# robustrobotics/flame

Hardware: AMD Instinct MI355X
Metric: NLTGV2 primal-dual iters/sec on 640x480 Delaunay graph; depth RMS vs CPU (higher is better)
Workload: dtype f32

## Files before the change

flame_amd/csrc/flame_nltgv2_test_options.h:

```cpp
#ifndef FLAME_NLTGV2_TEST_OPTIONS_H_
#define FLAME_NLTGV2_TEST_OPTIONS_H_

enum {
  FLAME_NLTGV2_OPT_BLOCK_WAVES = 103,
  FLAME_NLTGV2_OPT_UNROLL = 104,
  FLAME_NLTGV2_OPT_DUAL_PUBLISH = 106,
  FLAME_NLTGV2_OPT_PRESLEEP = 108,
  FLAME_NLTGV2_OPT_XCDS = 109,
  FLAME_NLTGV2_OPT_FAULT_INJECT = 110,
  FLAME_NLTGV2_OPT_POLL_GAP = 113
};

#endif
```

flame_amd/csrc/nltgv2_context.hip:

```cpp
#include "nltgv2_context.hpp"

namespace flame_hip {
namespace host {

int fail(flame_nltgv2_ctx* ctx, int status) {
  if (ctx) ctx->last_error = status;
  return status;
}

void request_open_stop(flame_nltgv2_ctx* ctx) {
  if (!ctx->open_inflight || ctx->open_stop_sent || !ctx->stop_dev.p || !ctx->ctl_stream) return;
  *ctx->h_stop = ctx->open_tag0;
  if (hipMemcpyAsync(ctx->stop_dev.p, ctx->h_stop, sizeof(unsigned), hipMemcpyHostToDevice, ctx->ctl_stream) != hipSuccess) (void)hipGetLastError();
  ctx->open_stop_sent = true;
}

hipError_t wait_solver_stream(flame_nltgv2_ctx* ctx) {
  request_open_stop(ctx);
  return hipStreamSynchronize(ctx->stream);
}

int ensure(flame_nltgv2_ctx* ctx, DevBuf& b, size_t bytes) {
  if (bytes == 0) bytes = 16;
  if (b.cap >= bytes) return 0;
// ... 442 lines not shown
  ok = ok && hipEventCreateWithFlags(&ctx->ev_snap, hipEventDisableTiming) == hipSuccess;
  ok = ok && hipEventCreateWithFlags(&ctx->ev_raster_done, hipEventDisableTiming) == hipSuccess;
  ok = ok && hipEventCreateWithFlags(&ctx->ev_topo_ready, hipEventDisableTiming) == hipSuccess;
  ok = ok && hipEventCreate(&ctx->ev_mesh0) == hipSuccess && hipEventCreate(&ctx->ev_mesh1) == hipSuccess;
  ok = ok && hipEventCreate(&ctx->ev_dbg0) == hipSuccess && hipEventCreate(&ctx->ev_dbg1) == hipSuccess;
  ok = ok && hipEventCreateWithFlags(&ctx->ev_expanded, hipEventDisableTiming) == hipSuccess;
  ok = ok && hipEventCreateWithFlags(&ctx->ev_run[0], hipEventDisableTiming) == hipSuccess;
  ok = ok && hipEventCreateWithFlags(&ctx->ev_run[1], hipEventDisableTiming) == hipSuccess;
  ok = ok && hipHostMalloc((void**)&ctx->h_err, kErrBytes, hipHostMallocDefault) == hipSuccess;
  ok = ok && hipHostMalloc((void**)&ctx->h_cost, 2 * sizeof(float), hipHostMallocDefault) == hipSuccess;
  ok = ok && hipHostMalloc((void**)&ctx->h_stop, 64, hipHostMallocDefault) == hipSuccess;
  if (ctx->h_stop) *ctx->h_stop = 0u;
  ok = ok && hipStreamCreateWithPriority(&ctx->ctl_stream, hipStreamNonBlocking, -1) == hipSuccess;
  if (!ok) {
    flame_nltgv2_destroy(ctx);
    return FLAME_NLTGV2_ERR_HIP;
  }
  ctx->stream = ctx->own_stream;
  *ctx->h_err = 0;
  {
    static std::once_flag warm;
    if (!std::getenv("FLAME_NLTGV2_NO_WARM"))
    std::call_once(warm, [ctx] {
      warm_module_kernels(), warm_module_persistent(ctx->own_stream, cooperative_allowed()), warm_module_persistent_tv(), warm_module_persistent_pv2();
      warm_module_layout(), warm_module_topo();
    });
    if (!std::getenv("FLAME_NLTGV2_LAZY_CALIBRATION") && ctx->prop.multiProcessorCount >= 64 && place_calibrate_at_create(device) && place_calibrate(ctx) != 0) {
      ctx->last_error = 0, ctx->last_hip = 0;
      (void)hipGetLastError();
    }
    if (ctx->place_state < 0) ctx->place_state = 0;
  }
  ctx->all = {&ctx->pos, &ctx->x, &ctx->w1, &ctx->w2, &ctx->xb, &ctx->w1b, &ctx->w2b, &ctx->xp, &ctx->w1p,
              &ctx->w2p, &ctx->data, &ctx->weight, &ctx->src, &ctx->dst, &ctx->alpha, &ctx->beta, &ctx->q1,
              &ctx->q2, &ctx->q3, &ctx->row_ptr, &ctx->half, &ctx->slice_row, &ctx->perm, &ctx->pdeg,
              &ctx->rec_nbr, &ctx->rec_edge, &ctx->edge_src_slot, &ctx->hrec, &ctx->hq, &ctx->vstate, &ctx->hq_alt, &ctx->vstate_alt, &ctx->cost_terms, &ctx->run_tail,
              &ctx->vaux, &ctx->bar0, &ctx->bar1, &ctx->vprev, &ctx->xbuf, &ctx->abort_flag, &ctx->tv_slot, &ctx->tv_vid, &ctx->tv_meta, &ctx->tv_wave, &ctx->wg2_slot, &ctx->wg2_vid, &ctx->wg2_meta, &ctx->wg2_nbr, &ctx->wg2_fetch, &ctx->wg2_info, &ctx->wg2_vfirst, &ctx->wg2_rmax, &ctx->err,
              &ctx->cost_out, &ctx->img_ref, &ctx->img_cmp, &ctx->photo_err, &ctx->r_tris, &ctx->r_valid, &ctx->r_tvalid, &ctx->r_keys,
              &ctx->r_img, &ctx->r_cov, &ctx->r_vtx, &ctx->r_val, &ctx->wg_slot, &ctx->wg_vid, &ctx->wg_meta, &ctx->wg_nbr,
              &ctx->wg_fetch, &ctx->wg_info, &ctx->wg_v0, &ctx->probe, &ctx->snap_hq, &ctx->snap_vstate, &ctx->snap_bar, &ctx->iperm,
              &ctx->order_m, &ctx->rid_of, &ctx->stage[0].d, &ctx->stage[1].d, &ctx->sync_init, &ctx->sync_vmap, &ctx->sync_emap, &ctx->sync_need,
              &ctx->wg_vfirst, &ctx->place_pool, &ctx->place_rank, &ctx->place_fill, &ctx->place_rec_off, &ctx->place_patch, &ctx->place_meas, &ctx->progress};
  for (DevBuf* b : {&ctx->feat_stamp_d, &ctx->feat_key_d, &ctx->feat_val_d, &ctx->topo_scratch, &ctx->topo_dims, &ctx->layout_pos}) ctx->all.push_back(b);
  for (auto& b : ctx->nx) ctx->all.push_back(&b);
  for (auto& b : ctx->ex) ctx->all.push_back(&b);
  ctx->all.push_back(&ctx->pos_undo);
  for (DevBuf* b : {&ctx->m_P, &ctx->m_idepth, &ctx->m_normals, &ctx->m_tvalid, &ctx->m_nvalid, &ctx->m_tnormal, &ctx->m_offset, &ctx->m_cursor,
// ... 89 lines not shown
      if (value != 2) ctx->persist_refused_topo = ctx->persist_backoff_topo = ~0ull;
      return 0;
    case FLAME_NLTGV2_OPT_PROBE:
      ctx->opt_probe = value ? 1 : 0;
      return 0;
    case FLAME_NLTGV2_OPT_DUAL_PUBLISH:
      if (value < 0 || value > 2) return fail(ctx, FLAME_NLTGV2_ERR_INVALID_ARG);
      ctx->opt_dual = value;
      return 0;
    case FLAME_NLTGV2_OPT_FAULT_INJECT:
      if (value < 0 || value > (1 << 24)) return fail(ctx, FLAME_NLTGV2_ERR_INVALID_ARG);
      ctx->opt_fault = value;
      if (value == 0) ctx->persist_refused_topo = ctx->persist_backoff_topo = ~0ull;
      return 0;
    case FLAME_NLTGV2_OPT_XCDS:
      if (value < 0 || value > 8) return fail(ctx, FLAME_NLTGV2_ERR_INVALID_ARG);
      ctx->opt_xcds = value;
      ctx->coop_checked_key = ~0ull;
      return 0;
    case FLAME_NLTGV2_OPT_PRESLEEP:
      if (value < 0 || value > 256) return fail(ctx, FLAME_NLTGV2_ERR_INVALID_ARG);
      ctx->opt_presleep = value;
      return 0;
    case FLAME_NLTGV2_OPT_MESH_STATE:
      if (value < 0 || value > 1) return fail(ctx, FLAME_NLTGV2_ERR_INVALID_ARG);
      ctx->opt_mesh_state = value;
      return 0;
    case FLAME_NLTGV2_OPT_COST_SUM:
      if (value < 0 || value > 1) return fail(ctx, FLAME_NLTGV2_ERR_INVALID_ARG);
      ctx->opt_cost_sum = value;
      return 0;
    case FLAME_NLTGV2_OPT_SYNC_PATH:
      if (value < 0 || value > 2) return fail(ctx, FLAME_NLTGV2_ERR_INVALID_ARG);
      ctx->opt_sync_path = value;
      return 0;
    case FLAME_NLTGV2_OPT_UNROLL:
      if (value != 0 && value != 4 && value != 8 && value != 16) return fail(ctx, FLAME_NLTGV2_ERR_INVALID_ARG);
      ctx->opt_unroll = value;
      return 0;
    default:
      return fail(ctx, FLAME_NLTGV2_ERR_INVALID_ARG);
  }
}


int flame_nltgv2_get_info(flame_nltgv2_ctx* ctx, flame_nltgv2_info* info) {
// ... 182 lines not shown
```

flame_amd/csrc/nltgv2_context.hpp:

```cpp
#ifndef FLAME_AMD_NLTGV2_CONTEXT_HPP_
#define FLAME_AMD_NLTGV2_CONTEXT_HPP_

#include <hip/hip_runtime.h>

#include <cstdio>
#include <cstdlib>
#include <cstring>
#include <algorithm>
#include <chrono>
#include <cmath>
#include <new>
#include <memory>
#include <mutex>
#include <functional>
#include <vector>

#include "flame_nltgv2.h"
#include "flame_nltgv2_test_options.h"
#include "nltgv2_kernels.h"
#include "nltgv2_pack.hpp"
#include "roctx_ranges.hpp"

namespace flame_hip {
namespace host {
// ... 106 lines not shown
  FlatMap feat_maps[3];
  int feat_cur = 0;
  bool feat_map_valid = false;
  std::vector<int32_t> feat_tab;
  std::vector<uint32_t> feat_stamp;
  uint32_t feat_stamp_now = 0;
  bool feat_tab_valid = false;
  int parity = 0;
  uint64_t topo = 0, stamp = 0;

  int opt_solver = 0, opt_use_graph = 1, opt_block_waves = 0, opt_unroll = 0, opt_persistent = 1, opt_dual = 1;
  int xbuf_form = 0;
  int opt_xcds = 0;
  bool photo_fused = false;
  PhotoGeometry photo_geo{};
  float photo_scale = 1.0f;
  int photo_border = 3;
  bool photo_fresh = false;
  float* export_ptr = nullptr;
  float export_scale = 1.0f;
  int opt_fault = 0;
  int opt_presleep = 0;
  int opt_poll_gap = 0;
  mutable int pv_occ = 0;
  mutable uint64_t pv_occ_topo = ~0ull;
  int opt_probe = 0;
  size_t probe_words = 0;
  uint32_t tag_next = 1;
  int last_run_path = 0, last_run_groups = 0;
  uint64_t persist_refused_topo = ~0ull;
  uint64_t persist_backoff_topo = ~0ull;
  int persist_backoff_left = 0, persist_timeout_streak = 0;
  int replaying = 0;
  uint64_t crowded_until_topo = 0;
  int last_run_waves_per_cu = 0;
  bool static_stale = false;
  uint64_t coop_checked_key = 0;
  int buf_gen = 0;
  int replay_attempt = 0;
  int replays_per_step = 0;
  int timeouts_recovered = 0;
  int torn_records_detected = 0;
  int opt_verify = 0;
  int opt_place = 1;
  int place_state = 0;
  uint64_t place_topo = ~0ull;
// ... 270 lines not shown
```

flame_amd/csrc/nltgv2_kernels.h:

```cpp
#pragma once

#include <hip/hip_runtime.h>
#include <hip/hip_ext.h>
#include <stdint.h>

namespace flame_hip {

struct SolverParams {
  float data_factor, step_x, step_q, theta, x_min, x_max;
};

struct PhotoGeometry {
  float KRKinv[9];
  float Kt[3];
};

struct PhotoFuse {
  const float2* pos = nullptr;
  const uint8_t* ref = nullptr;
  const uint8_t* cmp = nullptr;
  float* err = nullptr;
  PhotoGeometry geo{};
  float graph_scale = 1.0f;
  int rows = 0, cols = 0, step = 0, border = 0;
// ... 124 lines not shown
  const uint32_t* half = nullptr;
  const float2* pos = nullptr;
  float *alpha = nullptr, *beta = nullptr;
  uint8_t* need_nbr = nullptr;
};
int launch_sync_state(const SyncArgs& a, hipStream_t s);
int pv_patches_per_cu(const FusedArgs& a, bool verify);
struct Pv2Args {
  const int32_t* slot = nullptr;
  const int32_t* vid = nullptr;
  const uint32_t* meta = nullptr;
  const int32_t* nbr = nullptr;
  const int32_t* fetch = nullptr;
  const int32_t* info = nullptr;
  int count = 0, lcap = 0;
};
int launch_build_patches2(const CanonArgs& c, const FusedArgs& a, int n_patches, int32_t* wg_info, const int32_t* order_m, const int32_t* rid_tab,
                          const uint8_t* vfirst, const int32_t* iperm, int32_t* wg_slot, int32_t* wg_vid, uint32_t* wg_meta, int32_t* wg_nbr,
                          int32_t* wg_fetch, int* rmax, hipStream_t s);
int pv2_patches_per_cu(int lcap, bool verify);
int launch_persistent_pv2(const FusedArgs& a, const Pv2Args& w, const SolverParams& p, int wg_begin, int n_wgs, int parity_in, unsigned tag0,
                          int n_iters, unsigned max_spins, int poll_gap, int dual, const RunTail* tail, bool cooperative, hipStream_t stream);
int pv_real_waves_per_simd(bool verify_or_probe);
const void* persistent_tv_kernel(int waves_per_block, unsigned* lds_bytes);
int launch_build_sell(const CanonArgs& c, const FusedArgs& a, const int32_t* iperm, hipStream_t s);
int launch_build_patches(const CanonArgs& c, const FusedArgs& a, const int32_t* wg_v0, const int32_t* order_m,
                         const int32_t* rid_tab, const uint8_t* vfirst, const int32_t* iperm, hipStream_t s);
struct TopoDims {
  int32_t n_edges;
  int32_t n_keep;
  int32_t rows;
  int32_t max_degree;
  int32_t wg_count, wg_lcap;
  int32_t wg2_count, wg2_lcap;
  int32_t flags;
  int32_t pad_[7];
};
constexpr int32_t kTopoBadDegree = 1;
constexpr int32_t kTopoBadEdges = 2;
constexpr int kTopoInf = 0x7f7f7f7f;
struct TopoBuild {
  int V = 0, E = 0;
  int Vo = 0, Eo = 0;
  int n_slices = 0;
  const int32_t* fid = nullptr;
  const float2* pos = nullptr;
// ... 21 lines not shown
  void* sort_tmp = nullptr;
  size_t sort_tmp_bytes = 0;
  int* counters = nullptr;
  int32_t* old_of_new = nullptr;
  int32_t* old_of_new_edge = nullptr;
  int32_t *src = nullptr, *dst = nullptr;
  int32_t* row_ptr = nullptr;
  uint32_t* half = nullptr;
  int32_t *order_m = nullptr, *rid_of = nullptr, *perm = nullptr, *iperm = nullptr, *pdeg = nullptr, *slice_row = nullptr;
  int32_t *wg_info = nullptr, *wg_v0 = nullptr, *wg2_info = nullptr, *wg2_v0 = nullptr;
  uint8_t *wg_vfirst = nullptr, *wg2_vfirst = nullptr;
  TopoDims* dims = nullptr;
};
size_t topo_sort_temp_bytes(int V, int n_scan);
int launch_topo_feat_build(const int32_t* feat, int V, uint32_t* stamp, int32_t* key, int32_t* val, int tab_bits, uint32_t gen, hipStream_t s);
int launch_topo_sync_front(const TopoBuild& t, hipStream_t s);
int launch_topo_upload_front(const TopoBuild& t, hipStream_t s);
int launch_topo_back(const TopoBuild& t, hipStream_t s);

void warm_module_kernels();
void warm_module_persistent(hipStream_t stream, bool cooperative);
void warm_module_persistent_tv();
void warm_module_persistent_pv2();
void warm_module_layout();
void warm_module_topo();

int launch_save_prev(const CanonArgs& c, hipStream_t s);
int launch_dual(const CanonArgs& c, const SolverParams& p, hipStream_t s);
int launch_primal(const CanonArgs& c, const SolverParams& p, hipStream_t s);
int launch_extragradient(const CanonArgs& c, const SolverParams& p, hipStream_t s);
int launch_pack_static(const CanonArgs& c, const FusedArgs& a, hipStream_t s);
int launch_pack_state(const CanonArgs& c, const FusedArgs& a, int parity, bool with_static, hipStream_t s);
int launch_unpack_state(const CanonArgs& c, const FusedArgs& a, int parity, bool have_prev, hipStream_t s);
int launch_export(const CanonArgs& c, const FusedArgs& a, bool packed_current, float scale, float* dst,
                  hipStream_t s);
int launch_project_graph(const CanonArgs& c, float graph_scale, const ProjectGeometry& geo, uint8_t* keep, float2* pos_before, hipStream_t s);
int launch_rescale(const CanonArgs& c, float graph_scale, float* new_scale_dev, hipStream_t s);
int launch_interpolate_mesh(int T, const int32_t* tris, const float2* vtx, const float* values, float value_scale,
                            const uint8_t* vtx_valid, const uint8_t* tri_valid, unsigned long long* keys, float* img,
                            int* coverage, int rows, int cols, hipStream_t s);
int launch_photo_residual(const CanonArgs& c, float graph_scale, const PhotoGeometry& geo, const uint8_t* ref,
                          const uint8_t* cmp, int rows, int cols, int step, int border, float* err, hipStream_t s);
int launch_photo_residual_packed(const FusedArgs& a, const PhotoFuse& photo, hipStream_t s);
int launch_cost_terms(const CanonArgs& c, float* terms, hipStream_t s);
int launch_cost_sums(const CanonArgs& c, const float* terms, float* out2, hipStream_t s);

// ... 2 lines not shown
```

flame_amd/csrc/nltgv2_run.hip:

```cpp
#include "nltgv2_context.hpp"

namespace flame_hip {
namespace host {

void pick_config(const flame_nltgv2_ctx* ctx, int* unroll, int* wpb) {
  const bool small = ctx->L.n_slices <= 8 * ctx->prop.multiProcessorCount;
  *unroll = ctx->opt_unroll ? ctx->opt_unroll : (small ? 8 : 4);
  *wpb = ctx->opt_block_waves ? ctx->opt_block_waves : (small ? 1 : 4);
}

struct WaveGroup {
  int begin, count;
};

int ensure_form_rows(flame_nltgv2_ctx* ctx, int form);
int plan_groups(flame_nltgv2_ctx* ctx, int form, int total, int cap, const std::vector<int32_t>& cw, std::vector<WaveGroup>* groups);

bool cooperative_allowed() {
  static const bool ok = [] {
    if (std::getenv("FLAME_NLTGV2_NO_COOPERATIVE")) return false;
    if (std::getenv("FLAME_NLTGV2_COOPERATIVE")) return true;
    if (std::getenv("ROCP_TOOL_LIBRARIES")) return false;
    if (void* h = dlopen("librocprofiler-sdk.so.1", RTLD_NOLOAD | RTLD_LAZY)) {
      dlclose(h);
      return false;
    }
    return true;
  }();
  return ok;
}

int plan_persistent(flame_nltgv2_ctx* ctx, int n, std::vector<WaveGroup>* groups, bool consume = false) {
  groups->clear();
  if (!ctx->opt_persistent || n < 4 || n > (1 << 24) || !ctx->prop.cooperativeLaunch) return 0;
  if (ctx->persist_refused_topo == ctx->topo || ctx->replaying == 2) return 0;
  const bool retry = ctx->replaying == 1;
  if (!retry && ctx->persist_backoff_topo == ctx->topo && (ctx->persist_backoff_left > 0 || ctx->opt_fault > 0)) {
    if (consume && ctx->persist_backoff_left > 0) --ctx->persist_backoff_left;
    return 0;
  }
  PackedLayout& L = ctx->L;
  const int cus = ctx->prop.multiProcessorCount;
  const uint64_t occ_key = ctx->topo * 4 + (ctx->opt_verify != 0 ? 1 : 0) + (ctx->opt_probe != 0 ? 2 : 0);
  if (L.wg_ok && ctx->pv_occ_topo != occ_key) {
    ctx->pv_occ = std::min(kPvDensePerCu, pv_patches_per_cu(ctx->f, ctx->opt_verify != 0 || ctx->opt_probe != 0));
    if (std::getenv("FLAME_NLTGV2_TRACE"))
      std::fprintf(stderr, "[flame_nltgv2] pv: %d patches, row-packed %d, slab slots %d, local records %d -> %d resident per CU\n", L.wg_count,
                   (int)L.wg_rowpack, ctx->f.wg_slab_slots, ctx->f.wg_lcap, ctx->pv_occ);
    ctx->pv_occ_topo = occ_key;
  }
  const bool crowded = (ctx->topo < ctx->crowded_until_topo && ctx->opt_persistent == 1) || retry;
  const int wg_cap = (crowded ? std::min(ctx->pv_occ, kCrowdedWavesPerCu) : ctx->pv_occ) * cus;
  const bool pv_fits = L.wg_ok && L.wg_rowpack && L.wg_count > 0 && L.wg_count <= wg_cap;
  int form = 0;
  auto pv2_usable = [&]() -> bool {
    if (!ctx->wg2_built) return false;
    if (ctx->wg2_checked_topo != ctx->topo) {
// ... 374 lines not shown
    HIPCHK(ctx, hipEventRecord(ctx->ev_snap, ctx->stream));
    ctx->snap_topo = ctx->topo;
  }
  int rc = ensure_fused(ctx);
  if (rc) return rc;
  if (ctx->pending.active) {
    if (ctx->pending.ops.size() >= kMaxChain) {
      rc = finish(ctx);
    } else {
      rc = snapshot_chain_start(ctx);
    }
    if (rc) return rc;
  }
  int unroll, wpb;
  pick_config(ctx, &unroll, &wpb);
  std::vector<WaveGroup> groups;
  const int form = plan_persistent(ctx, n, &groups, true);
  const bool open_run = ctx->want_open != 0 && open_run_applies(ctx, form, groups) && !ctx->pending.active && ctx->opt_probe == 0 &&
                        ctx->opt_verify == 0 && ctx->replaying == 0 && (n & 1) == 0 && ctx->h_stop != nullptr && ctx->ctl_stream != nullptr;
  if (ctx->want_open != 0 && !open_run) {
    ctx->want_open = 0;
    return 0;
  }
  if (form != 0) {
    if ((uint64_t)ctx->tag_next + (uint64_t)n >= 0x07ff0000ull || (ctx->xbuf_form != 0 && ctx->xbuf_form != form)) {
      const size_t bytes = kXbufBytesPerVertex * records_capacity(ctx->L);
      HIPCHK(ctx, hipMemsetAsync(ctx->xbuf.p, 0, bytes, ctx->stream));
      if (ctx->place_base) {
        HIPCHK(ctx, hipMemsetAsync(ctx->place_base, 0, (size_t)2 * kPlacePages * 4096, ctx->stream));
        HIPCHK(ctx, hipMemsetAsync((int*)ctx->place_fill.p + 2 * kPlacePages, 0, 64, ctx->stream));
      }
      HIPCHK(ctx, hipMemsetAsync((int*)ctx->err.p + 12, 0, 2 * sizeof(int), ctx->stream));
      ctx->tag_next = 1;
    }
    ctx->xbuf_form = form;
    const uint32_t tag0 = ctx->tag_next + 2;
    const uint64_t key = ctx->topo * 1024 + (uint64_t)form * 64 + (ctx->opt_verify != 0 ? 16 : 0) + (ctx->opt_probe != 0 ? 8 : 0) +
                         (ctx->opt_dual == 2 ? 4 : ctx->opt_dual == 1 ? 2 : 0) + (ctx->opt_xcds > 0 ? 1 : 0);
    const RunTail* tail_dev = nullptr;
    {
      RunTail want;
      std::memset(static_cast<void*>(&want), 0, sizeof want);
      want.export_out = ctx->export_ptr, want.export_scale = ctx->export_scale;
      if (open_run) {
        const bool fresh = ctx->stop_dev.p == nullptr;
        rc = ensure(ctx, ctx->stop_dev, 64);
        if (rc) return rc;
        if (fresh) HIPCHK(ctx, hipMemsetAsync(ctx->stop_dev.p, 0, 64, ctx->stream));
        ctx->open_tag0 = tag0;
      }
      want.stop_req = open_run ? (const unsigned*)ctx->stop_dev.p : nullptr;
      const PhotoFuse pf = photo_target(ctx);
      std::memcpy(static_cast<void*>(&want.photo), &pf, sizeof pf);
      if (form == 3 && std::getenv("FLAME_NLTGV2_TRACE")) {
        rc = ensure(ctx, ctx->progress, 2 * sizeof(unsigned) * (size_t)ctx->L.wg_count);
        if (rc) return rc;
        HIPCHK(ctx, hipMemsetAsync(ctx->progress.p, 0, 2 * sizeof(unsigned) * (size_t)ctx->L.wg_count, ctx->stream));
        want.progress = (unsigned*)ctx->progress.p;
      }
      constexpr size_t kTailStride = (sizeof(RunTail) + 255) / 256 * 256;
      rc = ensure(ctx, ctx->run_tail, kTailStride * flame_nltgv2_ctx::kTailSlots);
// ... 46 lines not shown
          }
        }
        ctx->f.probe = nullptr;
        if (ctx->opt_probe) {
          const size_t words = (size_t)ctx->L.wg_count * (size_t)n * 8;
          rc = ensure(ctx, ctx->probe, words * sizeof(unsigned));
          if (rc) return rc;
          ctx->f.probe = (unsigned*)ctx->probe.p;
          ctx->probe_words = words;
          HIPCHK(ctx, hipMemsetAsync(ctx->probe.p, 0, words * sizeof(unsigned), ctx->stream));
        }
      }
      if (form == 4) {
        const bool dense = gr.count > kPv2PaceAbovePerCu * ctx->prop.multiProcessorCount;
        const int gap = ctx->opt_poll_gap > 0 ? ctx->opt_poll_gap - 1 : dense ? (3 | ((kPv2DenseGap - 1) << 4)) : kPvPollGap;
        const int poll_gap = gap | ((ctx->opt_presleep > 0 ? ctx->opt_presleep - 1 : dense ? kPv2DensePreSleep : kPvPreSleep) << 8);
        ctx->f.open_run = open_run ? 1 : 0;
        e = launch_persistent_pv2(ctx->f, ctx->pv2_args, to_sp(p), gr.begin, gr.count, ctx->parity, tag0, n, spins_arg, poll_gap, dual,
                                  tail_dev, cooperative_allowed() && ctx->coop_checked_key != key, ctx->stream);
        ctx->f.open_run = 0;
        if (e != 0) break;
        continue;
      }
      ctx->f.open_run = open_run ? 1 : 0;
      e = launch_persistent_run(ctx->f, to_sp(p), form, gr.begin, gr.count, ctx->parity, tag0, n, pw, spins_arg, presleep, dual,
                                xcds, tail_dev, cooperative_allowed() && ctx->coop_checked_key != key, ctx->stream);
      ctx->f.open_run = 0;
      if (e != 0) break;
    }
    ctx->run_event_bound = e == 0 && ctx->f.stop_event != nullptr;
    ctx->f.stop_event = nullptr;
    ctx->tag_next = tag0 + (uint32_t)n;
    if (e == 0) {
      if (!ctx->pending.active) {
        ctx->pending.active = true, ctx->pending.snapshotted = false;
        ctx->pending.ops.clear();
        ctx->pending.parity_before = ctx->parity, ctx->pending.have_prev_before = ctx->have_prev;
      }
      {
        flame_nltgv2_ctx::PendingOp op;
        op.kind = 0, op.params = *p, op.n = n;
        op.open = open_run, op.tag0 = tag0;
        op.dst = ctx->export_ptr, op.scale = ctx->export_scale;
        ctx->pending.ops.push_back(op);
      }
      ctx->photo_fresh = photo_target(ctx).err != nullptr;
// ... 405 lines not shown
```

flame_amd/regularizer.py:

```python
from __future__ import annotations

import ctypes as C
import os

import numpy as np

_HERE = os.path.dirname(os.path.abspath(__file__))
_LIB = None

_FP = C.POINTER(C.c_float)
_IP = C.POINTER(C.c_int32)

OPT_SOLVER, OPT_USE_HIPGRAPH, OPT_PERSISTENT, OPT_PROBE, OPT_VERIFY_RECORDS, OPT_PLACEMENT, OPT_SYNC_PATH, OPT_COST_SUM, OPT_MESH_STATE = 1, 2, 5, 12, 14, 16, 17, 18, 19
OPT_BLOCK_WAVES, OPT_UNROLL, OPT_DUAL_PUBLISH, OPT_PRESLEEP, OPT_XCDS, OPT_FAULT_INJECT, OPT_POLL_GAP = 103, 104, 106, 108, 109, 110, 113
RUN_PATHS = {0: "none", 1: "persistent (the lane-per-half-edge form, retired in round 3)", 2: "per-step hipGraph", 3: "per-step eager", 4: "canonical 4-sweep",
             5: "persistent-tv", 6: "persistent-pv", 7: "persistent-pv2"}
ERR_NAN = -5

VERTEX_STATE = ("x", "w1", "w2", "x_bar", "w1_bar", "w2_bar", "x_prev", "w1_prev", "w2_prev")
EDGE_STATE = ("q1", "q2", "q3")


def _rows_contiguous_u8(a) -> bool:
    return a.dtype == np.uint8 and a.ndim == 2 and a.strides[1] == 1 and a.strides[0] >= max(a.shape[1], 1)


class NLTGV2Error(RuntimeError):
    def __init__(self, status: int, what: str):
        super().__init__(f"{what}: status {status} ({status_string(status)})")
        self.status = status


class Params(C.Structure):

    _fields_ = [(n, C.c_float) for n in ("data_factor", "step_x", "step_q", "theta", "x_min", "x_max")]

    def __init__(self, data_factor=0.1, step_x=0.001, step_q=125.0, theta=0.25, x_min=0.0, x_max=10.0):
# ... 631 lines not shown
```

Baseline: 1.074 million.

## Add lean single-wave persistent PV kernel with inline-asm polling and DPP reductions

Adds a new persistent primal-dual kernel that runs one 64-lane wave per workgroup. The per-iteration loop is hand-written inline assembly: neighbour records are fetched with global_load_lds, readiness is polled on tags held in LDS, and the degree sums use DPP adds. The host selects it by default for form 3 when there is a single wave group, dual publish is on, max degree is at most 16 and occupancy allows. It is meant to cut the per-iteration synchronisation and instruction overhead of the generic persistent kernel. In exchange it adds a large hand-scheduled asm path that is hard to maintain, and correctness depends on its clobber lists and tag handling.

After: 1.142 million, median of 6. +6.3%, better.

```diff
diff --git a/flame_amd/csrc/flame_nltgv2_test_options.h b/flame_amd/csrc/flame_nltgv2_test_options.h
--- a/flame_amd/csrc/flame_nltgv2_test_options.h
+++ b/flame_amd/csrc/flame_nltgv2_test_options.h
@@ -8,7 +8,8 @@
   FLAME_NLTGV2_OPT_PRESLEEP = 108,
   FLAME_NLTGV2_OPT_XCDS = 109,
   FLAME_NLTGV2_OPT_FAULT_INJECT = 110,
-  FLAME_NLTGV2_OPT_POLL_GAP = 113
+  FLAME_NLTGV2_OPT_POLL_GAP = 113,
+  FLAME_NLTGV2_OPT_PV_LEAN = 114
 };
 
 #endif
diff --git a/flame_amd/csrc/nltgv2_context.hip b/flame_amd/csrc/nltgv2_context.hip
--- a/flame_amd/csrc/nltgv2_context.hip
+++ b/flame_amd/csrc/nltgv2_context.hip
@@ -488,7 +488,7 @@
     static std::once_flag warm;
     if (!std::getenv("FLAME_NLTGV2_NO_WARM"))
     std::call_once(warm, [ctx] {
-      warm_module_kernels(), warm_module_persistent(ctx->own_stream, cooperative_allowed()), warm_module_persistent_tv(), warm_module_persistent_pv2();
+      warm_module_kernels(), warm_module_persistent(ctx->own_stream, cooperative_allowed()), warm_module_persistent_tv(), warm_module_persistent_pv2(), warm_module_persistent_lean();
       warm_module_layout(), warm_module_topo();
     });
     if (!std::getenv("FLAME_NLTGV2_LAZY_CALIBRATION") && ctx->prop.multiProcessorCount >= 64 && place_calibrate_at_create(device) && place_calibrate(ctx) != 0) {
@@ -624,6 +624,10 @@
       if (value < 0 || value > 256) return fail(ctx, FLAME_NLTGV2_ERR_INVALID_ARG);
       ctx->opt_presleep = value;
       return 0;
+    case FLAME_NLTGV2_OPT_PV_LEAN:
+      if (value < 0 || value > 2) return fail(ctx, FLAME_NLTGV2_ERR_INVALID_ARG);
+      ctx->opt_pv_lean = value;
+      return 0;
     case FLAME_NLTGV2_OPT_MESH_STATE:
       if (value < 0 || value > 1) return fail(ctx, FLAME_NLTGV2_ERR_INVALID_ARG);
       ctx->opt_mesh_state = value;
diff --git a/flame_amd/csrc/nltgv2_context.hpp b/flame_amd/csrc/nltgv2_context.hpp
--- a/flame_amd/csrc/nltgv2_context.hpp
+++ b/flame_amd/csrc/nltgv2_context.hpp
@@ -152,6 +152,9 @@
   int opt_fault = 0;
   int opt_presleep = 0;
   int opt_poll_gap = 0;
+  int opt_pv_lean = 0;
+  mutable int pv_lean_occ = 0;
+  mutable uint64_t pv_lean_occ_topo = ~0ull;
   mutable int pv_occ = 0;
   mutable uint64_t pv_occ_topo = ~0ull;
   int opt_probe = 0;
diff --git a/flame_amd/csrc/nltgv2_kernels.h b/flame_amd/csrc/nltgv2_kernels.h
--- a/flame_amd/csrc/nltgv2_kernels.h
+++ b/flame_amd/csrc/nltgv2_kernels.h
@@ -170,6 +170,10 @@
 int launch_persistent_pv2(const FusedArgs& a, const Pv2Args& w, const SolverParams& p, int wg_begin, int n_wgs, int parity_in, unsigned tag0,
                           int n_iters, unsigned max_spins, int poll_gap, int dual, const RunTail* tail, bool cooperative, hipStream_t stream);
 int pv_real_waves_per_simd(bool verify_or_probe);
+int pv_lean_real_waves_per_simd();
+int pv_lean_patches_per_cu(const FusedArgs& a);
+int launch_persistent_pv_lean(const FusedArgs& a, const SolverParams& p, int wave_begin, int n_waves, int parity_in, unsigned tag0, int n_iters,
+                              unsigned max_spins, int xcds, const RunTail* tail, bool cooperative, hipStream_t stream);
 const void* persistent_tv_kernel(int waves_per_block, unsigned* lds_bytes);
 int launch_build_sell(const CanonArgs& c, const FusedArgs& a, const int32_t* iperm, hipStream_t s);
 int launch_build_patches(const CanonArgs& c, const FusedArgs& a, const int32_t* wg_v0, const int32_t* order_m,
@@ -237,6 +241,7 @@
 void warm_module_persistent(hipStream_t stream, bool cooperative);
 void warm_module_persistent_tv();
 void warm_module_persistent_pv2();
+void warm_module_persistent_lean();
 void warm_module_layout();
 void warm_module_topo();
 
diff --git a/flame_amd/csrc/nltgv2_persistent_lean.hip b/flame_amd/csrc/nltgv2_persistent_lean.hip
--- /dev/null
+++ b/flame_amd/csrc/nltgv2_persistent_lean.hip
@@ -0,0 +1,472 @@
+#include "nltgv2_persistent_common.hpp"
+
+namespace flame_hip {
+
+namespace {
+
+#define PVL_CLOBBERS                                                                                                                   \
+  "v64", "v65", "v66", "v67", "v68", "v69", "v70", "v71", "v72", "v73", "v74", "v75", "v76", "v77", "v78", "v79", "v80", "v81", "v82",  \
+      "v83", "v84", "v85", "v86", "v87", "v88", "v89", "v90", "v91", "v92", "v93", "v94", "v95", "v96", "v97", "v98", "v99", "v100",  \
+      "v101", "vcc", "scc", "memory"
+
+#define PVL_ADDS(J)                                                           \
+  "v_add_f32_dpp v84, v77, v84 row_shl:" #J " row_mask:0xf bank_mask:0xf\n\t" \
+  "v_add_f32_dpp v86, v80, v86 row_shl:" #J " row_mask:0xf bank_mask:0xf\n\t" \
+  "v_add_f32_dpp v87, v81, v87 row_shl:" #J " row_mask:0xf bank_mask:0xf\n\t" \
+  "v_add_f32_dpp v86, v82, v86 row_shl:" #J " row_mask:0xf bank_mask:0xf\n\t" \
+  "v_add_f32_dpp v87, v83, v87 row_shl:" #J " row_mask:0xf bank_mask:0xf\n\t"
+#define PVL_RM(J, M) "s_mov_b64 exec, %[" #M "]\n\t" PVL_ADDS(J)
+
+__global__ void __launch_bounds__(64)
+k_persistent_pv_lean(const int wg_begin, const int n_wgs, const int wgs_per_xcd, const int lcap, const int slab_slots,
+                     const int32_t* __restrict__ wg_slot, const int32_t* __restrict__ wg_vid,
+                     const uint32_t* __restrict__ wg_meta, const int32_t* __restrict__ wg_nbr,
+                     const int32_t* __restrict__ wg_fetch, const int32_t* __restrict__ wg_info, const int4* hrec,
+                     const float4* hq, const float4* vstate,
+                     float4* hq_out, float4* vstate_out, const float2* vaux, const float4* bar_in, float4* bar_out, float4* vprev,
+                     void* xbuf, const int rec_bytes, const int dual_arg, const unsigned tag0, const int n_iters,
+                     const unsigned max_spins_arg, const int poll_gap_arg, const SolverParams p,
+                     int* __restrict__ err, int* __restrict__ abort_flag, const int32_t* __restrict__ perm,
+                     const RunTail* __restrict__ tail, unsigned* __restrict__ probe, char* place_pool,
+                     const int32_t* __restrict__ rec_off, const int rec_off_stride, unsigned* rot_word) {
+  extern __shared__ float4 lds[];
+  constexpr int T = 64;
+  (void)dual_arg, (void)poll_gap_arg, (void)probe;
+  const unsigned max_spins = max_spins_arg & 0x7fffffffu;
+  const int lane = (int)threadIdx.x;
+  int b = blockIdx.x;
+  if (rot_word) {
+    const unsigned want = (tag0 & 0x0fffffffu) << 4;
+    if (b == 0 && lane == 0) __hip_atomic_store(rot_word, want | read_xcc_id(), __ATOMIC_RELAXED, __HIP_MEMORY_SCOPE_AGENT);
+    unsigned v = 0;
+    for (unsigned spins = 0;; ++spins) {
+      v = __builtin_amdgcn_readfirstlane(__hip_atomic_load(rot_word, __ATOMIC_RELAXED, __HIP_MEMORY_SCOPE_AGENT));
+      if ((v & ~15u) == want) break;
+      if (spins > (max_spins_arg & 0x7fffffffu)) {
+        if (lane == 0) {
+          give_up(abort_flag, err, false);
+          report_expired(err, 1, (int)blockIdx.x, -1, 0ull, -1, v, want);
+        }
+        return;
+      }
+      __builtin_amdgcn_s_sleep(2);
+    }
+    b += (int)(v & 7u);
+    if (b >= (int)gridDim.x) b -= (int)gridDim.x;
+  }
+  const int xcd = b & 7, idx = b >> 3;
+  if (idx >= wgs_per_xcd) return;
+  if (xcd * wgs_per_xcd + idx >= n_wgs) return;
+  const int wg = wg_begin + xcd * wgs_per_xcd + idx;
+  const int rid_base = wg_info[4 * wg], n_fetch = wg_info[4 * wg + 1];
+  const int count_flags = wg_info[4 * wg + 2];
+  if ((count_flags & 0xffff) == 0) return;
+  if (unsigned* const pg = tail->progress) {
+    if (lane == 0) pg[n_wgs + (wg - wg_begin)] = (unsigned)(wall_clock64() / 100u) | 1u;
+  }
+  const int stride = wg_info[4 * wg + 3];
+  const int rec_stride = lcap + T;
+  const int o_ovfA = 2 * rec_stride + slab_slots;
+  const __amdgpu_buffer_rsrc_t rx = make_rsrc(xbuf);
+  constexpr int kPar = 2;
+  const int S = rec_bytes, par = 2 * rec_bytes, tab_off = kPar * par;
+  const unsigned xcc_want = (tag0 & 0x0fffffffu) << 4;
+  const unsigned p0 = tag0 & 1u;
+
+  const size_t hl = (size_t)wg * T + lane;
+  const unsigned meta = wg_meta[hl];
+  const int slot = wg_slot[hl];
+  const int pv = wg_vid[hl];
+  const int nbr_code = wg_nbr[hl];
+  const int frid = (lane < n_fetch) ? wg_fetch[hl] : -1;
+  const int loc = (int)((meta >> 13) & 2047u);
+  const bool active = (meta & kWgActiveBit) != 0u;
+  const bool valid = (meta & kWgValidBit) != 0u, publishes = (meta & kWgPublishBit) != 0u;
+  const bool state_lane = (meta & kWgHeadBit) != 0u;
+  const unsigned degx = (meta & kWgHeadBit) ? ((meta >> 6) & 127u) : (active ? 255u : 0u);
+  const unsigned long long rm1 = __ballot(degx > 1u), rm2 = __ballot(degx > 2u), rm3 = __ballot(degx > 3u), rm4 = __ballot(degx > 4u),
+                           rm5 = __ballot(degx > 5u), rm6 = __ballot(degx > 6u), rm7 = __ballot(degx > 7u), rm8 = __ballot(degx > 8u);
+  const int nbr_idx = active ? ((nbr_code < 0) ? lcap + (nbr_code & 0x7fffffff) : nbr_code) : (valid ? loc : 0);
+
+  int4 rec = make_int4(0, 0, 0, 0);
+  float4 q = make_float4(0.f, 0.f, 0.f, 0.f);
+  if (active) {
+    rec = hrec[slot];
+    q = hq[slot];
+  }
+  const bool is_target = rec.x < 0;
+  const float alpha = __int_as_float(rec.y), dx = __int_as_float(rec.z), dy = __int_as_float(rec.w);
+  const float beta = q.w;
+  float q1 = q.x;
+  v2f_t q23 = {q.y, q.z};
+  const float as = is_target ? -alpha : alpha, bs = is_target ? -beta : beta, ac = is_target ? alpha : -alpha;
+  const v2f_t P12 = {alpha * dx, alpha * dy};
+  const v2f_t C2 = !active ? v2f_t{0.0f, 0.0f} : is_target ? v2f_t{beta, beta} : v2f_t{-dx, -dy};
+  const float nbeta = -beta;
+  const v2f_t bs2 = {bs, bs}, nbeta2 = {nbeta, nbeta};
+
+  float4 st = make_float4(0.f, 0.f, 0.f, 0.f), bs4 = make_float4(0.f, 0.f, 0.f, 0.f);
+  float2 aux = make_float2(0.f, 0.f);
+  if (valid) {
+    st = vstate[pv];
+    aux = vaux[pv];
+    bs4 = bar_in[pv];
+  }
+  const float data = st.w;
+  const float thr = p.step_x * (p.data_factor * aux.x);
+  float x = st.x;
+  v2f_t w12 = {st.y, st.z};
+  float xb = bs4.x;
+  v2f_t wb12 = {bs4.y, bs4.z};
+  float x_prev = x;
+  v2f_t w_prev = w12;
+  bool timed_out = n_fetch > T;
+
+  const int my_off = (rid_base + loc) << 4;
+  const int rec_w = valid ? loc : o_ovfA + lane, rec_wstride = valid ? rec_stride : 0;
+
+  lds[lcap + lane] = make_float4(0.f, 0.f, 0.f, 0.f);
+  lds[rec_stride + lcap + lane] = make_float4(0.f, 0.f, 0.f, 0.f);
+
+  int off0 = (frid >= 0) ? (frid << 4) : 0;
+  bool fetch_remote = frid >= 0;
+  {
+    const unsigned my_xcc = read_xcc_id();
+    if (state_lane && publishes)
+      __builtin_amdgcn_raw_buffer_store_b32((int)(xcc_want | my_xcc), rx, tab_off + (my_off >> 2), 0, kAuxSc1);
+    if (n_fetch > 0 && !timed_out) {
+      bool pend = frid >= 0;
+      unsigned g0 = 0, spins = 0;
+      for (;;) {
+        if (pend) {
+          int o = tab_off + (frid << 2);
+          asm volatile("" : "+v"(o)::"memory");
+          g0 = (unsigned)__builtin_amdgcn_raw_buffer_load_b32(rx, o, 0, kAuxSc1);
+          pend = ((g0 & ~15u) != xcc_want);
+        }
+        if (!__any(pend)) break;
+        if (++spins > max_spins) {
+          timed_out = true;
+          const unsigned long long pm = __ballot(pend);
+          const int fl = __ffsll((long long)pm) - 1;
+          const int ff = __shfl(frid, fl, 64);
+          const unsigned gs = (unsigned)__shfl((int)g0, fl, 64);
+          if (lane == 0) report_expired(err, 2, wg, -1, pm, ff, gs, xcc_want);
+          break;
+        }
+        __builtin_amdgcn_s_sleep(2);
+      }
+      if (!timed_out && frid >= 0 && (g0 & 15u) == my_xcc) off0 += S, fetch_remote = false;
+    }
+  }
+  const unsigned long long fetch_mask = __ballot(frid >= 0);
+  const bool pub_lane = state_lane && publishes;
+  const char* const xb_base = static_cast<const char*>(xbuf);
+  const bool placed = place_pool != nullptr;
+  int pub0 = -1, pub1 = -1;
+  const char* src0 = xb_base + off0;
+  const char* src1 = xb_base + off0 + par;
+  if (placed) {
+    if (pub_lane) pub0 = rec_off[rid_base + loc], pub1 = rec_off[rec_off_stride + rid_base + loc];
+    if (fetch_remote) {
+      const int o0 = rec_off[frid], o1 = rec_off[rec_off_stride + frid];
+      if (o0 >= 0) src0 = place_pool + o0;
+      if (o1 >= 0) src1 = place_pool + o1;
+    }
+  }
+  char* const xb_w = static_cast<char*>(xbuf);
+  char* const pa0 = pub0 >= 0 ? place_pool + pub0 : xb_w + my_off;
+  char* const pa1 = pub1 >= 0 ? place_pool + pub1 : xb_w + my_off + par;
+  char* const la0 = xb_w + my_off + S;
+  char* const la1 = xb_w + my_off + S + par;
+  {
+    lds[(p0 ? rec_wstride : 0) + rec_w] = make_float4(xb, wb12.x, wb12.y, __uint_as_float(tag0));
+    if (pub_lane) {
+      v4i_t o;
+      o.x = __float_as_int(xb), o.y = __float_as_int(wb12.x), o.z = __float_as_int(wb12.y), o.w = (int)tag0;
+      asm volatile("global_store_dwordx4 %0, %1, off sc1\n\t"
+                   "global_store_dwordx4 %2, %1, off" ::"v"(p0 ? pa1 : pa0), "v"(o), "v"(p0 ? la1 : la0) : "memory");
+    }
+  }
+  lds_wave_sync();
+  const unsigned lds_addr0 = (unsigned)(size_t)(lds);
+
+  const unsigned long long it_mask = __ballot(is_target), pub_mask = __ballot(pub_lane), rec_mask = __ballot(state_lane || !valid);
+  const unsigned u_sq = __float_as_uint(p.step_q), u_sx = __float_as_uint(p.step_x), u_th = __float_as_uint(p.theta);
+  const unsigned long long sq2 = ((unsigned long long)u_sq << 32) | u_sq, sx2 = ((unsigned long long)u_sx << 32) | u_sx,
+                           th2 = ((unsigned long long)u_th << 32) | u_th;
+  const float x_min_v = p.x_min, x_max_v = p.x_max;
+  const float neg_zero = -0.0f;
+  unsigned ok_lane = 1u;
+
+  auto step = [&](const unsigned s, const unsigned rd_nbr, const unsigned dst, const unsigned rd_own, const unsigned wr_own, const int it,
+                  const char* const src, char* const pub_r, char* const pub_l) {
+    const unsigned own_slot = dst + 16u * (unsigned)lane;
+    const unsigned s_next = s + 1u;
+    {
+      unsigned cnt, keep, pend_lo, tag_seen, outer, ab;
+      unsigned long long pnarrow, exec_saved, t64a, t64b;
+      asm volatile("s_branch 0f\n\t"
+                   "5:\n\t"
+                   PVL_RM(8, m8) PVL_ADDS(9)
+                   "s_cmp_le_u32 %[md], 10\n\t"
+                   "s_cbranch_scc1 6f\n\t"
+                   PVL_ADDS(10) PVL_ADDS(11)
+                   "s_cmp_le_u32 %[md], 12\n\t"
+                   "s_cbranch_scc1 6f\n\t"
+                   PVL_ADDS(12)
+                   "s_cmp_le_u32 %[md], 13\n\t"
+                   "s_cbranch_scc1 6f\n\t"
+                   PVL_ADDS(13)
+                   "s_cmp_le_u32 %[md], 14\n\t"
+                   "s_cbranch_scc1 6f\n\t"
+                   PVL_ADDS(14) PVL_ADDS(15)
+                   "s_branch 6f\n\t"
+                   "0:\n\t"
+                   "ds_read_b32 v67, %[ro]\n\t"
+                   "ds_read2_b32 v[70:71], %[ro] offset0:1 offset1:2\n\t"
+                   "v_mov_b32 v95, %[tagn]\n\t"
+                   "s_setprio 0\n\t"
+                   "s_mov_b64 %[ex], exec\n\t"
+                   "s_mov_b32 %[keep], m0\n\t"
+                   "s_mov_b32 m0, %[dst]\n\t"
+                   "s_mov_b32 %[cnt], 0\n\t"
+                   "s_mov_b32 %[outer], 0\n\t"
+                   "s_mov_b64 %[pn], %[fm]\n\t"
+                   "1:\n\t"
+                   "s_mov_b64 exec, %[pn]\n\t"
+                   "global_load_lds_dwordx4 %[src], off sc1\n\t"
+                   "s_mov_b64 exec, %[ex]\n\t"
+                   "ds_read_b32 v64, %[ra] offset:12\n\t"
+                   "ds_read_b32 v65, %[fa] offset:12\n\t"
+                   "ds_read_b32 v66, %[ra]\n\t"
+                   "ds_read2_b32 v[68:69], %[ra] offset0:1 offset1:2\n\t"
+                   "s_add_u32 %[cnt], %[cnt], 1\n\t"
+                   "s_waitcnt lgkmcnt(0)\n\t"
+                   "v_cmp_ne_u32_e32 vcc, %[tag], v65\n\t"
+                   "s_and_b64 %[pn], vcc, %[fm]\n\t"
+                   "v_cmp_ne_u32_e32 vcc, %[tag], v64\n\t"
+                   "s_cmp_lt_u32 %[cnt], 64\n\t"
+                   "s_cbranch_vccz 2f\n\t"
+                   "s_cbranch_scc1 1b\n\t"
+                   "v_mov_b32 v97, 0\n\t"
+                   "global_load_dword v97, v97, %[abp] sc1\n\t"
+                   "s_waitcnt vmcnt(0)\n\t"
+                   "v_readfirstlane_b32 %[ab], v97\n\t"
+                   "s_add_u32 %[outer], %[outer], 1\n\t"
+                   "s_cmp_lg_u32 %[ab], 0\n\t"
+                   "s_cbranch_scc1 7f\n\t"
+                   "s_mov_b32 %[cnt], 0\n\t"
+                   "s_cmp_le_u32 %[outer], %[omax]\n\t"
+                   "s_cbranch_scc1 1b\n\t"
+                   "7:\n\t"
+                   "s_or_b32 %[pl], vcc_lo, vcc_hi\n\t"
+                   "v_mov_b32 %[tv], v64\n\t"
+                   "s_branch 8f\n\t"
+                   "2:\n\t"
+                   "s_setprio 3\n\t"
+                   "v_sub_f32 v76, v67, v66\n\t"
+                   "v_pk_add_f32 v[72:73], v[70:71], v[68:69] neg_lo:[0,1] neg_hi:[0,1]\n\t"
+                   "v_cndmask_b32_e64 v75, v71, v69, %[itm]\n\t"
+                   "v_cndmask_b32_e64 v74, v70, v68, %[itm]\n\t"
+                   "v_mul_f32 v76, %[as], v76\n\t"
+                   "v_pk_mul_f32 v[74:75], %[P12], v[74:75]\n\t"
+                   "v_pk_mul_f32 v[72:73], %[bs2], v[72:73]\n\t"
+                   "v_sub_f32 v76, v76, v74\n\t"
+                   "v_sub_f32 v76, v76, v75\n\t"
+                   "v_mul_f32 v76, %[sq], v76\n\t"
+                   "v_add_f32 v96, %[q1], v76\n\t"
+                   "v_pk_mul_f32 v[72:73], %[sq2], v[72:73]\n\t"
+                   "v_med3_f32 %[q1], v96, -1.0, 1.0\n\t"
+                   "v_pk_add_f32 v[98:99], %[q23], v[72:73]\n\t"
+                   "v_mul_f32 v77, %[sx], %[q1]\n\t"
+                   "v_med3_f32 v100, v98, -1.0, 1.0\n\t"
+                   "v_med3_f32 v101, v99, -1.0, 1.0\n\t"
+                   "v_pk_mul_f32 v[78:79], %[sx2], v[100:101]\n\t"
+                   "v_mul_f32 v77, %[ac], v77\n\t"
+                   "v_cndmask_b32_e64 v81, v77, v79, %[itm]\n\t"
+                   "v_cndmask_b32_e64 v80, v77, v78, %[itm]\n\t"
+                   "v_pk_mul_f32 v[80:81], %[C2], v[80:81]\n\t"
+                   "v_pk_mul_f32 v[82:83], %[nb2], v[78:79]\n\t"
+                   "v_pk_add_f32 v[86:87], %[w12], v[80:81]\n\t"
+                   "v_cndmask_b32_e64 v83, v83, %[nz], %[itm]\n\t"
+                   "v_cndmask_b32_e64 v82, v82, %[nz], %[itm]\n\t"
+                   "v_pk_add_f32 v[86:87], v[82:83], v[86:87]\n\t"
+                   "v_add_f32 v84, %[x], v77\n\t"
+                   PVL_RM(1, m1) PVL_RM(2, m2) PVL_RM(3, m3) PVL_RM(4, m4) PVL_RM(5, m5) PVL_RM(6, m6) PVL_RM(7, m7)
+                   "s_cmp_gt_u32 %[md], 8\n\t"
+                   "s_cbranch_scc1 5b\n\t"
+                   "6:\n\t"
+                   "s_mov_b64 exec, %[ex]\n\t"
+                   "v_sub_f32 v85, v84, %[dat]\n\t"
+                   "v_add_f32 v90, %[thr], v84\n\t"
+                   "v_cmp_lt_f32_e64 vcc, v85, -%[thr]\n\t"
+                   "v_sub_f32 v91, v84, %[thr]\n\t"
+                   "v_pk_add_f32 v[88:89], v[86:87], %[w12] neg_lo:[0,1] neg_hi:[0,1]\n\t"
+                   "v_cndmask_b32_e32 v90, %[dat], v90, vcc\n\t"
+                   "v_cmp_gt_f32_e32 vcc, v85, %[thr]\n\t"
+                   "v_pk_mul_f32 v[88:89], %[th2], v[88:89]\n\t"
+                   "v_mov_b64 %[wp], %[w12]\n\t"
+                   "v_cndmask_b32_e32 v90, v90, v91, vcc\n\t"
+                   "v_cmp_gt_f32_e32 vcc, %[xmn], v90\n\t"
+                   "v_add_f32 v93, v86, v88\n\t"
+                   "v_add_f32 v94, v87, v89\n\t"
+                   "v_cndmask_b32_e32 v90, v90, %[xmnv], vcc\n\t"
+                   "v_cmp_lt_f32_e32 vcc, %[xmx], v90\n\t"
+                   "v_mov_b64 %[w12], v[86:87]\n\t"
+                   "v_mov_b32 %[xp], %[x]\n\t"
+                   "v_cndmask_b32_e32 v91, v90, %[xmxv], vcc\n\t"
+                   "v_sub_f32 v85, v91, %[x]\n\t"
+                   "v_mul_f32 v85, %[th], v85\n\t"
+                   "v_add_f32 v85, v91, v85\n\t"
+                   "v_cmp_gt_f32_e32 vcc, %[xmn], v85\n\t"
+                   "v_mov_b32 %[x], v91\n\t"
+                   "v_mov_b64 %[q23], v[100:101]\n\t"
+                   "v_cndmask_b32_e32 v85, v85, %[xmnv], vcc\n\t"
+                   "v_cmp_lt_f32_e32 vcc, %[xmx], v85\n\t"
+                   "v_cmp_le_f32_e64 %[ta], |v96|, %[fmx]\n\t"
+                   "v_cmp_le_f32_e64 %[tb], |v98|, %[fmx]\n\t"
+                   "v_cndmask_b32_e32 v92, v85, %[xmxv], vcc\n\t"
+                   "s_mov_b64 exec, %[pubm]\n\t"
+                   "global_store_dwordx4 %[pr], v[92:95], off sc1\n\t"
+                   "global_store_dwordx4 %[pl2], v[92:95], off\n\t"
+                   "s_mov_b64 exec, %[recm]\n\t"
+                   "s_setprio 0\n\t"
+                   "ds_write_b128 %[wo], v[92:95]\n\t"
+                   "s_mov_b64 exec, %[ex]\n\t"
+                   "v_cndmask_b32_e64 %[ok], 0, %[ok], %[ta]\n\t"
+                   "v_cmp_le_f32_e64 %[ta], |v99|, %[fmx]\n\t"
+                   "v_cndmask_b32_e64 %[ok], 0, %[ok], %[tb]\n\t"
+                   "s_mov_b32 %[pl], 0\n\t"
+                   "v_cndmask_b32_e64 %[ok], 0, %[ok], %[ta]\n\t"
+                   "8:\n\t"
+                   "s_mov_b32 m0, %[keep]"
+                   : [keep] "=&s"(keep), [cnt] "=&s"(cnt), [pl] "=&s"(pend_lo), [pn] "=&s"(pnarrow), [ex] "=&s"(exec_saved), [ta] "=&s"(t64a),
+                     [tb] "=&s"(t64b), [outer] "=&s"(outer), [ab] "=&s"(ab), [tv] "=&v"(tag_seen), [ok] "+v"(ok_lane), [q1] "+v"(q1), [q23] "+v"(q23), [x] "+v"(x), [w12] "+v"(w12),
+                     [xp] "+v"(x_prev), [wp] "+v"(w_prev)
+                   : [src] "v"(src), [dst] "s"(dst), [ra] "v"(rd_nbr), [fa] "v"(own_slot), [ro] "v"(rd_own), [wo] "v"(wr_own), [pr] "v"(pub_r),
+                     [pl2] "v"(pub_l), [tag] "s"(s), [tagn] "s"(s_next), [fm] "s"(fetch_mask), [itm] "s"(it_mask), [pubm] "s"(pub_mask),
+                     [recm] "s"(rec_mask), [as] "v"(as), [P12] "v"(P12), [bs2] "v"(bs2), [ac] "v"(ac), [C2] "v"(C2), [nb2] "v"(nbeta2),
+                     [nz] "v"(neg_zero), [dat] "v"(data), [thr] "v"(thr), [xmnv] "v"(x_min_v), [xmxv] "v"(x_max_v), [sq] "s"(p.step_q),
+                     [sq2] "s"(sq2), [sx] "s"(p.step_x), [sx2] "s"(sx2), [th] "s"(p.theta), [th2] "s"(th2), [xmn] "s"(p.x_min), [xmx] "s"(p.x_max),
+                     [fmx] "s"(3.402823466e+38f), [abp] "s"(abort_flag), [omax] "s"(max_spins >> 4), [md] "s"(stride), [m1] "s"(rm1), [m2] "s"(rm2), [m3] "s"(rm3), [m4] "s"(rm4), [m5] "s"(rm5),
+                     [m6] "s"(rm6), [m7] "s"(rm7), [m8] "s"(rm8)
+                   : PVL_CLOBBERS);
+      if (__builtin_expect(__builtin_amdgcn_readfirstlane(pend_lo) != 0u, 0)) {
+        timed_out = true;
+        if (__builtin_amdgcn_readfirstlane(ab) == 0u) {
+          const unsigned long long pm = __ballot(tag_seen != s);
+          const int fl = __ffsll((long long)pm) - 1;
+          const int ni = __shfl(nbr_idx, fl, 64);
+          const int ff = ni >= lcap ? __shfl(frid, ni - lcap, 64) : -2 - ni;
+          const unsigned gs = (unsigned)__shfl((int)tag_seen, fl, 64);
+          if (lane == 0) report_expired(err, 3, wg, it, pm, ff, gs, s);
+        }
+      }
+    }
+  };
+
+  const int areaA = p0 ? rec_stride : 0, areaB = p0 ? 0 : rec_stride;
+  const unsigned rdA_nbr = lds_addr0 + 16u * (unsigned)(areaA + nbr_idx), rdB_nbr = lds_addr0 + 16u * (unsigned)(areaB + nbr_idx);
+  const unsigned dstA = __builtin_amdgcn_readfirstlane(lds_addr0 + 16u * (unsigned)(areaA + lcap));
+  const unsigned dstB = __builtin_amdgcn_readfirstlane(lds_addr0 + 16u * (unsigned)(areaB + lcap));
+  const int wrA_rec = (valid ? areaA : 0) + rec_w, wrB_rec = (valid ? areaB : 0) + rec_w;
+  const unsigned ownA = lds_addr0 + 16u * (unsigned)wrA_rec, ownB = lds_addr0 + 16u * (unsigned)wrB_rec;
+  const char* const srcA = p0 ? src1 : src0;
+  const char* const srcB = p0 ? src0 : src1;
+  char* const pubA = p0 ? pa1 : pa0;
+  char* const pubB = p0 ? pa0 : pa1;
+  char* const locA = p0 ? la1 : la0;
+  char* const locB = p0 ? la0 : la1;
+  int it = 0;
+  for (; it + 1 < n_iters && !timed_out; it += 2) {
+    step(tag0 + (unsigned)it, rdA_nbr, dstA, ownA, ownB, it, srcA, pubB, locB);
+    if (timed_out) break;
+    step(tag0 + (unsigned)it + 1u, rdB_nbr, dstB, ownB, ownA, it + 1, srcB, pubA, locA);
+  }
+  if (it < n_iters && !timed_out) step(tag0 + (unsigned)it, rdA_nbr, dstA, ownA, ownB, it, srcA, pubB, locB);
+  asm volatile("s_waitcnt vmcnt(0)" ::: "memory");
+
+  if (timed_out) {
+    if (lane == 0) {
+      give_up(abort_flag, err, false);
+      unsigned* const pg = tail->progress;
+      if (pg) pg[wg - wg_begin] = 0x80000000u | (unsigned)(it + 1);
+    }
+    return;
+  }
+
+  const float4 last = lds[(n_iters & 1) ? wrB_rec : wrA_rec];
+  xb = last.x, wb12 = v2f_t{last.y, last.z};
+  if (state_lane) write_back_vertex(pv, x, w12, xb, wb12, x_prev, w_prev, data, vstate_out, bar_out, vprev, perm, tail);
+  if (active) hq_out[slot] = make_float4(q1, q23.x, q23.y, beta);
+  if (ok_lane == 0u && active) atomicOr(err, 1);
+}
+
+#undef PVL_RM
+#undef PVL_ADDS
+#undef PVL_CLOBBERS
+
+unsigned pv_lean_lds_bytes(int lcap, int slab_slots) { return 16u * (unsigned)(2 * (lcap + 64) + slab_slots + 64); }
+
+}
+
+int pv_lean_real_waves_per_simd() {
+  return 4;
+}
+
+int pv_lean_patches_per_cu(const FusedArgs& a) {
+  if (!a.wg_rowpack) return 0;
+  int n = 0;
+  if (hipOccupancyMaxActiveBlocksPerMultiprocessor(&n, (const void*)k_persistent_pv_lean, 64, pv_lean_lds_bytes(a.wg_lcap, a.wg_slab_slots)) != hipSuccess) {
+    (void)hipGetLastError();
+    return 0;
+  }
+  return n < 4 * pv_lean_real_waves_per_simd() ? n : 4 * pv_lean_real_waves_per_simd();
+}
+
+int launch_persistent_pv_lean(const FusedArgs& a, const SolverParams& p, int wave_begin, int n_waves, int parity_in, unsigned tag0, int n_iters,
+                              unsigned max_spins, int xcds, const RunTail* tail, bool cooperative, hipStream_t stream) {
+  if (n_waves <= 0 || n_iters <= 0) return (int)hipSuccess;
+  if (!a.wg_rowpack) return (int)hipErrorInvalidConfiguration;
+  if (xcds < 1 || xcds > 8) xcds = 8;
+  int wgx = (n_waves + xcds - 1) / xcds;
+  const dim3 gv((unsigned)(wgx * 8)), bv(64u);
+  int lcap = a.wg_lcap, slab_slots = a.wg_slab_slots, poll_gap = a.wg_poll_gap, dual = 1;
+  const int32_t *w0 = a.wg_slot, *w1 = a.wg_vid, *w3 = a.wg_nbr, *w4 = a.wg_fetch, *w5 = a.wg_info;
+  const uint32_t* w2 = a.wg_meta;
+  const int4* hrec = a.hrec;
+  const float4* hq = a.hq;
+  const float4* vstate = a.vstate;
+  float4* hq_out = a.hq_out;
+  float4* vstate_out = a.vstate_out;
+  const float2* vaux = a.vaux;
+  const float4* bin = a.bar[parity_in];
+  float4* bout = a.bar[parity_in ^ 1];
+  float4* vprev = a.vprev;
+  void* xbuf = a.xbuf;
+  int rec_bytes = persistent_rec_bytes(a);
+  SolverParams pp = p;
+  int* err = a.err;
+  int* abort_flag = a.abort_flag;
+  const int32_t* perm = a.perm;
+  unsigned* probe = nullptr;
+  char* place_pool = (a.rec_off && wave_begin == 0 && xcds == 8) ? a.place_pool : nullptr;
+  const int32_t* rec_off = a.rec_off;
+  int rec_off_stride = a.rec_off_stride;
+  unsigned* rot_word = place_pool ? a.rot_word : nullptr;
+  const unsigned ldsv = pv_lean_lds_bytes(lcap, slab_slots);
+  void* vargs[] = {&wave_begin, &n_waves, &wgx, &lcap, &slab_slots, &w0, &w1, &w2, &w3, &w4, &w5, &hrec, &hq, &vstate,
+                   &hq_out, &vstate_out, &vaux, &bin, &bout, &vprev, &xbuf, &rec_bytes, &dual, &tag0, &n_iters,
+                   &max_spins, &poll_gap, &pp, &err, &abort_flag, &perm, &tail, &probe, &place_pool, &rec_off, &rec_off_stride, &rot_word};
+  const void* fv = (const void*)k_persistent_pv_lean;
+  if (cooperative) return (int)hipLaunchCooperativeKernel(fv, gv, bv, vargs, ldsv, stream);
+  return (int)hipExtLaunchKernel(fv, gv, bv, vargs, ldsv, stream, nullptr, a.stop_event, 0);
+}
+
+void warm_module_persistent_lean() {
+  hipFuncAttributes fa;
+  if (hipFuncGetAttributes(&fa, (const void*)k_persistent_pv_lean) != hipSuccess) (void)hipGetLastError();
+}
+
+}
diff --git a/flame_amd/csrc/nltgv2_run.hip b/flame_amd/csrc/nltgv2_run.hip
--- a/flame_amd/csrc/nltgv2_run.hip
+++ b/flame_amd/csrc/nltgv2_run.hip
@@ -30,9 +30,21 @@
   return ok;
 }
 
+static bool pv_lean_applies(const flame_nltgv2_ctx* ctx, int form, const std::vector<WaveGroup>& groups, bool open_run) {
+  if (form != 3 || groups.size() != 1 || ctx->opt_pv_lean == 1) return false;
+  if (ctx->opt_probe != 0 || ctx->opt_verify != 0 || open_run || ctx->replaying != 0 || ctx->opt_fault != 0) return false;
+  if (ctx->opt_poll_gap != 0 || ctx->opt_presleep != 0) return false;
+  const int cus = ctx->prop.multiProcessorCount, count = groups[0].count;
+  const bool dual_on = ctx->opt_dual == 2 || (ctx->opt_dual == 1 && count > kDualMinWavesPerCu * cus);
+  if (!dual_on || count > kPvPaceAbovePerCu * cus) return false;
+  if (ctx->L.max_degree > 16 || !ctx->L.wg_rowpack) return false;
+  if (ctx->pv_lean_occ_topo != ctx->topo) ctx->pv_lean_occ = pv_lean_patches_per_cu(ctx->f), ctx->pv_lean_occ_topo = ctx->topo;
+  return count <= ctx->pv_lean_occ * cus;
+}
+
 int plan_persistent(flame_nltgv2_ctx* ctx, int n, std::vector<WaveGroup>* groups, bool consume = false) {
   groups->clear();
-  if (!ctx->opt_persistent || n < 4 || n > (1 << 24) || !ctx->prop.cooperativeLaunch) return 0;
+  if (!ctx->opt_persistent || n < (ctx->opt_pv_lean == 2 ? 1 : 4) || n > (1 << 24) || !ctx->prop.cooperativeLaunch) return 0;
   if (ctx->persist_refused_topo == ctx->topo || ctx->replaying == 2) return 0;
   const bool retry = ctx->replaying == 1;
   if (!retry && ctx->persist_backoff_topo == ctx->topo && (ctx->persist_backoff_left > 0 || ctx->opt_fault > 0)) {
@@ -453,6 +465,8 @@
     ctx->want_open = 0;
     return 0;
   }
+  const bool lean = pv_lean_applies(ctx, form, groups, open_run);
+  if (ctx->opt_pv_lean == 2 && !lean) return fail(ctx, FLAME_NLTGV2_ERR_INVALID_ARG);
   if (form != 0) {
     if ((uint64_t)ctx->tag_next + (uint64_t)n >= 0x07ff0000ull || (ctx->xbuf_form != 0 && ctx->xbuf_form != form)) {
       const size_t bytes = kXbufBytesPerVertex * records_capacity(ctx->L);
@@ -467,7 +481,7 @@
     ctx->xbuf_form = form;
     const uint32_t tag0 = ctx->tag_next + 2;
     const uint64_t key = ctx->topo * 1024 + (uint64_t)form * 64 + (ctx->opt_verify != 0 ? 16 : 0) + (ctx->opt_probe != 0 ? 8 : 0) +
-                         (ctx->opt_dual == 2 ? 4 : ctx->opt_dual == 1 ? 2 : 0) + (ctx->opt_xcds > 0 ? 1 : 0);
+                         (ctx->opt_dual == 2 ? 4 : ctx->opt_dual == 1 ? 2 : 0) + (ctx->opt_xcds > 0 ? 1 : 0) + (lean ? 32 : 0);
     const RunTail* tail_dev = nullptr;
     {
       RunTail want;
@@ -560,6 +574,12 @@
         if (e != 0) break;
         continue;
       }
+      if (lean) {
+        e = launch_persistent_pv_lean(ctx->f, to_sp(p), gr.begin, gr.count, ctx->parity, tag0, n, spins_arg, xcds, tail_dev,
+                                      cooperative_allowed() && ctx->coop_checked_key != key, ctx->stream);
+        if (e != 0) break;
+        continue;
+      }
       ctx->f.open_run = open_run ? 1 : 0;
       e = launch_persistent_run(ctx->f, to_sp(p), form, gr.begin, gr.count, ctx->parity, tag0, n, pw, spins_arg, presleep, dual,
                                 xcds, tail_dev, cooperative_allowed() && ctx->coop_checked_key != key, ctx->stream);
diff --git a/flame_amd/regularizer.py b/flame_amd/regularizer.py
--- a/flame_amd/regularizer.py
+++ b/flame_amd/regularizer.py
@@ -12,7 +12,7 @@
 _IP = C.POINTER(C.c_int32)
 
 OPT_SOLVER, OPT_USE_HIPGRAPH, OPT_PERSISTENT, OPT_PROBE, OPT_VERIFY_RECORDS, OPT_PLACEMENT, OPT_SYNC_PATH, OPT_COST_SUM, OPT_MESH_STATE = 1, 2, 5, 12, 14, 16, 17, 18, 19
-OPT_BLOCK_WAVES, OPT_UNROLL, OPT_DUAL_PUBLISH, OPT_PRESLEEP, OPT_XCDS, OPT_FAULT_INJECT, OPT_POLL_GAP = 103, 104, 106, 108, 109, 110, 113
+OPT_BLOCK_WAVES, OPT_UNROLL, OPT_DUAL_PUBLISH, OPT_PRESLEEP, OPT_XCDS, OPT_FAULT_INJECT, OPT_POLL_GAP, OPT_PV_LEAN = 103, 104, 106, 108, 109, 110, 113, 114
 RUN_PATHS = {0: "none", 1: "persistent (the lane-per-half-edge form, retired in round 3)", 2: "per-step hipGraph", 3: "per-step eager", 4: "canonical 4-sweep",
              5: "persistent-tv", 6: "persistent-pv", 7: "persistent-pv2"}
 ERR_NAN = -5
```
